# NTU-CompHydroMet-Lab/P2I-GAN-benchmark

Hardware: AMD Instinct MI355X
Metric: train frames/sec (128x128x16) (higher is better)
Workload: dtype f32

## Files before the change

### include/p2i_hip.h

```cpp
#ifndef P2I_HIP_H
#define P2I_HIP_H
#include <stdint.h>

#ifdef __cplusplus
extern "C" {
#endif

#define P2I_OK 0
#define P2I_EINVAL (-1)
#define P2I_ELDS (-2)

#define P2I_ACT_NONE 0
#define P2I_ACT_RELU 1
#define P2I_ACT_LEAKY 2
#define P2I_ACT_TANH 3

int p2i_abi_version(void);
const char* p2i_last_error(void);

typedef struct {
  int B, Cin, Cout;
  int Ti, Hi, Wi;
  int To, Ho, Wo;
  int kt, kh, kw;
// ... 4 lines not shown
int p2i_conv_fwd(const p2i_conv_desc* d, const float* x, const float* wp, const float* bias,
                 const float* residual, float* y, int act, void* stream);
int p2i_conv_dgrad(const p2i_conv_desc* d, const float* dy, const float* y_act, int act,
                   const float* wp_d, const float* dx_add, const float* mask_y, int mask_act,
                   float* dx, void* stream);
int p2i_conv_wgrad(const p2i_conv_desc* d, const float* x, const float* dy, const float* y_act,
                   int act, float* dwp, float* dbias, void* stream);
int p2i_conv_wgrad_ws(const p2i_conv_desc* d, const float* x, const float* dy, const float* y_act, int act, float* dwp,
                      float* dbias, float* ws, int64_t ws_floats, void* stream);
int p2i_conv_fwd_x6(const p2i_conv_desc* d, const float* x, const float* wp, uint16_t* wsplit, const float* bias,
                    const float* residual, float* y, int act, void* stream);
int p2i_conv_dgrad_x6(const p2i_conv_desc* d, const float* dy, const float* wp_d, uint16_t* wsplit, const float* dx_add,
                      const float* mask_y, int mask_act, float* dx, void* stream);
int p2i_x6_split(const float* wp, uint16_t* wb, int ntaps, int K, int Mpad, void* stream);
int p2i_x6_split_batched(const float* const* wp, uint16_t* const* wb, const int* ntaps, const int* K, const int* Mpad, int n,
                         void* stream);
int p2i_x6c_would_take(const p2i_conv_desc* d, int dgrad, int act);
int p2i_conv_fwd_x6s(const p2i_conv_desc* d, const float* x, const float* wp, const uint16_t* wb_layer, int ntaps_w,
                     const float* bias, const float* residual, float* y, int act, void* stream);
int p2i_conv_dgrad_x6s(const p2i_conv_desc* d, const float* dy, const float* wp_d, const uint16_t* wb_layer, int ntaps_w,
                       const float* dx_add, const float* mask_y, int mask_act, float* dx, void* stream);
int p2i_conv_last_plan(int* out6);
int p2i_fast_div_magic(int d, uint32_t* magic);
int p2i_wgrad_last_plan(int* out4);

int p2i_doconv_fold_fwd(const float* W, const float* D, const float* D_diag, int O, int I, int groups,
                        int ksz, int identity_rep, float* wp_f, float* wp_d, void* stream);
int p2i_doconv_fold_bwd(const float* dwp_f, const float* W, const float* D, const float* D_diag,
                        int O, int I, int groups, int ksz, float* dW, float* dD, void* stream);

int p2i_doconv_fold_fwd_batched(const float* const* W, const float* const* D, const float* const* D_diag, int n, int O, int I,
                                float* const* wp_f, float* const* wp_d, void* stream);
int p2i_doconv_fold_bwd_batched(const float* const* dwp_f, const float* const* W, const float* const* D,
                                const float* const* D_diag, int n, int O, int I, float* const* dW, float* const* dD,
                                void* stream);

int p2i_weight_pack(const float* w, int O, int I, int ntaps, const float* inv_div_ptr,
                    float* wp_f, float* wp_d, void* stream);
int p2i_weight_unpack_grad(const float* dwp_f, int O, int I, int ntaps, const float* w_orig,
                           const float* sigma_ptr, const float* u, const float* v, float* scratch,
                           float* dw, void* stream);

int p2i_weight_pack_batched(const float* const* w, const int* O, const int* I, const int* ntaps, const float* const* inv_div,
                            float* const* wp_f, float* const* wp_d, int n, void* stream);
int p2i_weight_unpack_grad_batched(const float* const* dwp_f, const int* O, const int* I, const int* ntaps,
                                   const float* const* w_orig, const float* const* sigma, const float* const* u,
// ... 284 lines not shown
```

### p2i-gan-benchmark_amd/csrc/conv_x6c.hip

```cpp
#include "conv_common.h"

namespace p2i {

#ifdef P2I_STAMP
extern __device__ unsigned long long* p2i_stamp_buf;
#define X6C_NOW(v) do { __builtin_amdgcn_sched_barrier(0); asm volatile("s_memtime %0\n\ts_waitcnt lgkmcnt(0)" : "=s"(v) :: "memory"); __builtin_amdgcn_sched_barrier(0); } while (0)
#define X6C_ACC(sum, t_prev) do { unsigned long long t_; X6C_NOW(t_); sum += t_ - t_prev; t_prev = t_; } while (0)
#else
#define X6C_NOW(v) do { } while (0)
#define X6C_ACC(sum, t_prev) do { } while (0)
#endif

typedef __bf16 bf16x8c __attribute__((ext_vector_type(8)));
typedef unsigned u32x4c __attribute__((ext_vector_type(4)));

__device__ __forceinline__ unsigned pack_hi16c(float lo_elem, float hi_elem) {
  return __builtin_amdgcn_perm(__float_as_uint(hi_elem), __float_as_uint(lo_elem), 0x07060302u);
}
__device__ __forceinline__ float trunc_bf16c(float v) { return __uint_as_float(__float_as_uint(v) & 0xFFFF0000u); }
__device__ __forceinline__ void split8c(const float (&v)[8], u32x4c& hi, u32x4c& mid, u32x4c& lo) {
#pragma unroll
  for (int j = 0; j < 4; ++j) {
    const float a = v[2 * j], b = v[2 * j + 1];
    hi[j] = pack_hi16c(a, b);
// ... 63 lines not shown
  const int blocks = total > 0 ? (total + 255) / 256 : 1;
  P2I_LAUNCH(wsplit_kernel, dim3(blocks > 2048 ? 2048 : blocks), dim3(256), 0, s, wp, reinterpret_cast<u32x4c*>(wb), ntaps, Ck, CmPad);
  return launch_status();
}

struct X6cGeom {
  const float* src; float* dst; const uint16_t* wb; const float* bias; const float* res; const float* mask_y;
  unsigned wb_bytes;
  int act_epi, mask_act;
  int B, Ck, Cm, CmPad;
  int sH, sW, dT, dH, dW, nH, nW;
  int ljb, ljh, ljw, eH, eW, CSl, bH, bW, nth, ntw;
  unsigned mg_ew, mg_eh;
  int ntaps_w, ksplit;
  int sT, nT, mT, oT, pT, ns, sdt0, sdt1, sdt2, swt0, swt1, swt2;
  int tap_off[9];
  int tap_w[9];
  int fused_atomic;
  int stagger;
  int vec4_epi;
  const u32x4c* splanes;
  unsigned plane_units;
  int cons_prio;
};

__device__ constexpr int X6C_CLS[9] = {3, 3, 3, 3, 2, 2, 1, 1, 0};

template <int NW> struct X6cTile {
  static constexpr int MAXCSL = NW == 8 ? 384 : 256;
  static constexpr int NI = (2 * MAXCSL + 64 * NW - 1) / (64 * NW);
};

#define X6C_WAIT1(b) asm volatile("s_waitcnt vmcnt(%0)" ::"n"(b) : "memory")
#define X6C_WAIT2(b) if (n < (b) + 1) { X6C_WAIT1(b); } else { X6C_WAIT1((b) + 1); }
#define X6C_WAIT4(b) if (n < (b) + 2) { X6C_WAIT2(b) } else { X6C_WAIT2((b) + 2) }
#define X6C_WAIT8(b) if (n < (b) + 4) { X6C_WAIT4(b) } else { X6C_WAIT4((b) + 4) }
#define X6C_WAIT16(b) if (n < (b) + 8) { X6C_WAIT8(b) } else { X6C_WAIT8((b) + 8) }
#define X6C_WAIT32(b) if (n < (b) + 16) { X6C_WAIT16(b) } else { X6C_WAIT16((b) + 16) }
__device__ __forceinline__ void x6c_wait_vm(int n) {
  if (n < 0 || n > 62) n = 0;
  if (n < 32) { X6C_WAIT32(0) } else { X6C_WAIT32(32) }
}

template <int NW, int TM, bool FUSED = false, int TPS = 3>
__global__ __launch_bounds__(64 * NW) void patch_gemm_x6c_kernel(const X6cGeom g) {
  constexpr int NCLS = FUSED ? 4 : 1;
  constexpr int NSTG = 9 / TPS;
// ... 300 lines not shown
#endif
}


template <int TM, int TPS, bool FUSED = false, bool EPI4 = false, int NPW = 4, int TN = 2, bool PRE = false>
__global__ __launch_bounds__(64 * (4 + NPW)) void patch_gemm_x6p_kernel(const X6cGeom g) {
  constexpr int NSTG = 9 / TPS;
  constexpr int NCLS = FUSED ? 4 : 1;
  static_assert(TPS == 3 || TPS == 9, "taps per stage");
  extern __shared__ __attribute__((aligned(16))) float smem[];
  constexpr int MB = 32 * TM, NCW = 4, NTHR = 64 * (NCW + NPW), NPT = 64 * NPW;
  constexpr int NI = (2 * (TN == 2 ? X6cTile<8>::MAXCSL : X6cTile<4>::MAXCSL) + NPT - 1) / NPT;
  constexpr int RING = TPS == 9 ? 3 : (TM == 2 ? 4 : 6), LEAD = RING - 1;
  constexpr int WST = 6 * TPS * MB, NWI = WST / 64;
  const int CSl = g.CSl;
  int* ptab = reinterpret_cast<int*>(smem);
  const int ptab_sz = (CSl + 3) & ~3;
  u32x4c* wbuf = reinterpret_cast<u32x4c*>(smem + ptab_sz);
  u32x4c* planes = wbuf + RING * WST;
  const int PST = 6 * CSl;

  const int tid = threadIdx.x, lane = tid & 63, wave = __builtin_amdgcn_readfirstlane(tid >> 6);
  const int l31 = lane & 31, lhi = lane >> 5;
  int tile = blockIdx.x;
  const int tw = tile % g.ntw; tile /= g.ntw;
  const int th = tile % g.nth;
  const int tb = tile / g.nth;
  const int j0b = tb << g.ljb, j0h = th << g.ljh, j0w = tw << g.ljw;
  const int o0 = blockIdx.y * MB;
  const int JWm = (1 << g.ljw) - 1, JHm = (1 << g.ljh) - 1;
  const int sHW = g.sH * g.sW;
  const int src_h0 = j0h + g.bH, src_w0 = j0w + g.bW;
  const int KCt = g.Ck >> 3;
  const int cps = g.Ck >> 4;
  const int cs = g.sT * sHW;
  const int nimg = g.B * g.nT;
  const int c0 = blockIdx.z * ((g.ns * cps) / g.ksplit);
  const int nch = (g.ns * cps) / g.ksplit;
  const int nst = NSTG * nch;

  for (int e = tid; e < CSl; e += NTHR) {
    const int row = fast_div(e, g.mg_ew);
    const int ew = e - row * g.eW;
    const int jb = fast_div(row, g.mg_eh);
    const int eh = row - jb * g.eH;
    const int n = j0b + jb, h = src_h0 + eh, w = src_w0 + ew;
    const int b = n / g.nT, lt = n - b * g.nT;
    ptab[e] = (n < nimg && (unsigned)h < (unsigned)g.sH && (unsigned)w < (unsigned)g.sW) ? ((b * (PRE ? KCt : g.Ck)) * g.sT + lt * g.mT) * sHW + h * g.sW + w : -1;
  }
  __syncthreads();

#ifdef P2I_STAMP
// ... 398 lines not shown
#ifdef P2I_STAMP
  if (p2i_stamp_buf && lane == 0) {
    asm volatile("s_waitcnt vmcnt(0)" ::: "memory");
    unsigned long long st_end; X6C_NOW(st_end);
    unsigned long long* o = p2i_stamp_buf + ((size_t)(blockIdx.x + gridDim.x * blockIdx.y) * 8 + wave) * 8;
    o[0] = st_a; o[1] = st_d; o[2] = st_b; o[3] = st_c; o[4] = st_l1 - st_l0; o[5] = st_l0 - st_entry; o[6] = st_e; o[7] = st_end - st_l1;
  }
#endif
}

static bool x6c_on() { return P2I_ENV_ONCE("P2I_CONV_X6C", 1) != 0; }
static bool x6c_fused_on() { return P2I_ENV_ONCE("P2I_CONV_X6C_FUSED", 1) != 0; }
static int x6c_min_wg() { return env_int("P2I_X6C_MIN_WG", 200); }
static int x6c_min_wg_low() { return env_int("P2I_X6C_MIN_WG", env_int("P2I_X6C_MIN_WG_LOW", 64)); }
static int x6c_fused_min_wg() { return env_int("P2I_X6C_MIN_WG", 128); }
static int x6p_tn1() { return env_int("P2I_X6P_TN1", 1); }
static int x6c_forced() { return env_int("P2I_X6C_TILE", 0); }
static int x6c_stagger() { return env_int("P2I_X6C_STAGGER", 0); }
static int x6c_fused_ksplit() { return env_int("P2I_X6C_FUSED_KSPLIT", 0); }
static int x6p_npw() { return env_int("P2I_X6P_NPW", 8) == 4 ? 4 : 8; }
static int x6c_pc() { return env_int("P2I_X6C_PC", 1); }
static int x6c_tps1() { return env_int("P2I_X6C_TPS", 9) == 3 ? 3 : 9; }
static int x6p_prio() { return env_int("P2I_X6P_PRIO", 0); }

struct X6cVariant { int NW, TM; };
static const X6cVariant kX6cVariants[] = {{8, 2}, {8, 1}, {4, 1}};

struct X6cPick { int v, jb, jh, jw, csl, ksplit; long long wgs; };
static X6cPick x6c_pick(int B, int nH, int nW, int Cm, int Ck, bool linear_epi, int Ck_slice) {
  int forced = x6c_forced();
  const int min_wg = x6c_min_wg();
  const bool tn1_ok = x6c_pc() && Ck_slice >= 32;
  if (forced == 41 && !tn1_ok) forced = 81;
  const int ksplit_on = P2I_ENV_ONCE("P2I_X6C_KSPLIT", 1);
  static const int order_a[5][2] = {{0, 0}, {1, 0}, {2, 0}, {1, 1}, {0, 1}}, order_b[5][2] = {{0, 0}, {0, 1}, {1, 0}, {2, 0}, {1, 1}};
  X6cPick low{-1, 0, 0, 0, 0, 1, 0};
  for (int cand = 0; cand < 5; ++cand) {
      const int v = (ksplit_on == 2 ? order_b : order_a)[cand][0], pass = (ksplit_on == 2 ? order_b : order_a)[cand][1];
      const X6cVariant& t = kX6cVariants[v];
      if (v == 2 && (!tn1_ok || (forced ? forced != 41 : !x6p_tn1()))) continue;
      if (forced && forced != t.NW * 10 + t.TM) continue;
      if (t.TM == 2 && Cm <= 32 && !forced) continue;
      if (pass == 1 && ((ksplit_on != 2 && t.TM != 1) || !ksplit_on || !linear_epi || ((Ck >> 4) & 1) || forced)) continue;
      int jb, jt, jh, jw;
      pick_tile_dims(32 * t.NW, B, 1, nH, nW, jb, jt, jh, jw);
      const int csl = jb * (jh + 2) * (jw + 2);
// ... 73 lines not shown
  k.wb_bytes = (2u * (unsigned)ntaps_w + (unsigned)tw_max + 1u) * (unsigned)g.Ck * (unsigned)g.CmPad * 2u;
  k.act_epi = g.act_epi; k.mask_act = g.mask_act;
  k.B = g.B; k.Ck = g.Ck; k.Cm = g.Cm; k.CmPad = g.CmPad;
  k.sH = g.sH; k.sW = g.sW; k.dT = g.dT; k.dH = g.dH; k.dW = g.dW; k.nH = c0.nH; k.nW = c0.nW;
  k.ljb = ilog2(pk.jb); k.ljh = ilog2(pk.jh); k.ljw = ilog2(pk.jw);
  k.eH = pk.jh + halo; k.eW = pk.jw + halo; k.CSl = pk.csl;
  k.nth = ceil_div(c0.nH, pk.jh); k.ntw = ceil_div(c0.nW, pk.jw);
  k.mg_ew = magic_u16(k.eW); k.mg_eh = magic_u16(k.eH);
  k.ntaps_w = ntaps_w; k.ksplit = pk.ksplit;
  k.sT = g.sT; k.nT = c0.nT; k.mT = c0.mT; k.oT = c0.oT; k.pT = c0.pT; k.ns = ns;
  k.stagger = x6c_stagger(); k.cons_prio = x6p_prio();
  return k;
}

template <void (*KERN)(const X6cGeom), int NTHR>
static void x6c_launch(const X6cGeom& k, dim3 grid, size_t lds, hipStream_t s) {
  static bool attr_set = false;
  if (!attr_set) {
    (void)hipFuncSetAttribute((const void*)KERN, hipFuncAttributeMaxDynamicSharedMemorySize, 160 * 1024);
    attr_set = true;
  }
  P2I_LAUNCH(KERN, grid, dim3(NTHR), lds, s, k);
}
static void x6c_dispatch(const X6cGeom& k, const X6cVariant& tv, int tps, bool fused, int* plan6, hipStream_t s) {
  const size_t lds = x6c_lds_bytes(k.CSl, tv.TM, tps);
  const dim3 grid((unsigned)(ceil_div(k.B * k.nT, 1 << k.ljb) * k.nth * k.ntw), (unsigned)ceil_div(k.Cm, 32 * tv.TM), (unsigned)k.ksplit);
  const bool pc = x6c_pc() && k.Ck >= 32 && (!fused || tps == 9);
  if (plan6) { plan6[0] = 32 * tv.TM; plan6[1] = 32 * tv.NW; plan6[2] = k.ksplit; plan6[3] = pc ? 4 : 8; plan6[4] = tps; plan6[5] = fused ? 8 : 7; }
  const bool pre = k.splanes != nullptr;
  if (!fused && pc) {
    if (tv.TM == 2) {
      if (k.vec4_epi) x6c_launch<patch_gemm_x6p_kernel<2, 3, false, true>, 512>(k, grid, lds, s);
      else x6c_launch<patch_gemm_x6p_kernel<2, 3>, 512>(k, grid, lds, s);
    } else if (tv.NW == 4) {
      if (pre) x6c_launch<patch_gemm_x6p_kernel<1, 9, false, false, 8, 1, true>, 768>(k, grid, lds, s);
      else x6c_launch<patch_gemm_x6p_kernel<1, 9, false, false, 8, 1>, 768>(k, grid, lds, s);
    } else if (tps == 9) {
      if (pre && x6p_npw() == 8) x6c_launch<patch_gemm_x6p_kernel<1, 9, false, false, 8, 2, true>, 768>(k, grid, lds, s);
      else if (x6p_npw() == 8) x6c_launch<patch_gemm_x6p_kernel<1, 9, false, false, 8>, 768>(k, grid, lds, s);
      else x6c_launch<patch_gemm_x6p_kernel<1, 9>, 512>(k, grid, lds, s);
    } else x6c_launch<patch_gemm_x6p_kernel<1, 3>, 512>(k, grid, lds, s);
  } else if (!fused) {
    if (tv.TM == 2) x6c_launch<patch_gemm_x6c_kernel<8, 2>, 512>(k, grid, lds, s);
    else if (tps == 9) x6c_launch<patch_gemm_x6c_kernel<8, 1, false, 9>, 512>(k, grid, lds, s);
    else x6c_launch<patch_gemm_x6c_kernel<8, 1>, 512>(k, grid, lds, s);
  } else if (pc) x6c_launch<patch_gemm_x6p_kernel<1, 9, true>, 512>(k, grid, lds, s);
  else if (tps == 9) x6c_launch<patch_gemm_x6c_kernel<8, 1, true, 9>, 512>(k, grid, lds, s);
  else x6c_launch<patch_gemm_x6c_kernel<8, 1, true>, 512>(k, grid, lds, s);
}

// ... 123 lines not shown
  for (int i = 0; i < n; ++i) {
    P2I_REQUIRE(wp[i] && wb[i] && ntaps[i] > 0 && K[i] > 0 && (K[i] & 7) == 0 && Mpad[i] > 0 && (Mpad[i] & 31) == 0, "p2i_x6_split_batched: bad tensor %d", i);
    b.wp[i] = wp[i]; b.wb[i] = reinterpret_cast<u32x4c*>(wb[i]); b.ntaps[i] = ntaps[i]; b.Ck[i] = K[i]; b.CmPad[i] = Mpad[i];
    const int tot = ntaps[i] * (K[i] >> 3) * Mpad[i];
    if (tot > maxn) maxn = tot;
  }
  const int blocks = (maxn + 255) / 256;
  P2I_LAUNCH(wsplit_batched_kernel, dim3(blocks > 1024 ? 1024 : blocks, n), dim3(256), 0, (hipStream_t)stream, b);
  return launch_status();
}

extern "C" int p2i_x6_split_planes(const float* x, void* planes, int B, int C, int64_t P, void* stream) {
  P2I_REQUIRE(x && planes && B > 0 && C > 0 && (C & 7) == 0 && P > 0, "split planes: C % 8 == 0");
  const long long total = (long long)B * (C >> 3) * P;
  const long long blocks = (total + 255) / 256;
  P2I_LAUNCH(p2i::split_planes_kernel, dim3((unsigned)(blocks > 8192 ? 8192 : blocks)), dim3(256), 0, (hipStream_t)stream, x,
             static_cast<p2i::u32x4c*>(planes), B, C >> 3, (long long)P);
  return p2i::launch_status();
}
extern "C" int p2i_x6_next_source_planes(const void* planes) {
  p2i::g_next_splanes = planes;
  return P2I_OK;
}
```

### p2i-gan-benchmark_amd/csrc/wgrad_x6.hip

```cpp
#include "conv_common.h"

namespace p2i {

#ifdef P2I_STAMP
extern __device__ unsigned long long* p2i_stamp_buf;
#define WX_NOW(v) do { __builtin_amdgcn_sched_barrier(0); asm volatile("s_memtime %0\n\ts_waitcnt lgkmcnt(0)" : "=s"(v) :: "memory"); __builtin_amdgcn_sched_barrier(0); } while (0)
#else
#define WX_NOW(v) do { } while (0)
#endif

typedef short s16x4w __attribute__((ext_vector_type(4)));
typedef __bf16 bf16x8w __attribute__((ext_vector_type(8)));
typedef unsigned u32x4w __attribute__((ext_vector_type(4)));
typedef float f32x4w __attribute__((ext_vector_type(4)));

struct Wx6Geom {
  const float* x;
  const float* dy;
  float* dwp;
  float* partial;
  float* dbias;
  long long pstride;
  long long bias_off;
  int B, Cx, Co, CoPad, H, W;
// ... 18 lines not shown
#pragma unroll
  for (int j = 0; j < 4; ++j) {
    const float a = v[2 * j], b = v[2 * j + 1];
    hi[j] = wx_pack(a, b);
    const float ra = a - wx_trunc(a), rb = b - wx_trunc(b);
    mid[j] = wx_pack(ra, rb);
    const float sa = ra - wx_trunc(ra), sb = rb - wx_trunc(rb);
    lo[j] = wx_pack(sa, sb);
  }
}

typedef __attribute__((address_space(3))) s16x4w* lds_s16x4_ptr;
__device__ __forceinline__ bf16x8w wx_read_tr(const unsigned char* base, int byte_off) {
  const s16x4w a = __builtin_amdgcn_ds_read_tr16_b64_v4i16((lds_s16x4_ptr)(base + byte_off));
  const s16x4w b = __builtin_amdgcn_ds_read_tr16_b64_v4i16((lds_s16x4_ptr)(base + byte_off + 4 * WX_ROW));
  return __builtin_bit_cast(bf16x8w, __builtin_shufflevector(a, b, 0, 1, 2, 3, 4, 5, 6, 7));
}
__device__ __forceinline__ bf16x8w wx_read_tr_s4(const unsigned char* base, int byte_off) {
  const s16x4w a = __builtin_amdgcn_ds_read_tr16_b64_v4i16((lds_s16x4_ptr)(base + byte_off));
  const s16x4w b = __builtin_amdgcn_ds_read_tr16_b64_v4i16((lds_s16x4_ptr)(base + byte_off + WX_ROW));
  return __builtin_bit_cast(bf16x8w, __builtin_shufflevector(a, b, 0, 1, 2, 3, 4, 5, 6, 7));
}

template <bool S4, int DIAG = 0>
__global__ __launch_bounds__(512) void wgrad_x6_kernel(const Wx6Geom g) {
  extern __shared__ __attribute__((aligned(16))) unsigned char wsm[];
#ifdef P2I_STAMP
  unsigned long long st_entry, st_loop0 = 0, st_loop1 = 0, st_bar = 0, st_t;
  WX_NOW(st_entry);
#endif
  const int tid = threadIdx.x, lane = tid & 63, wave = __builtin_amdgcn_readfirstlane(tid >> 6);
  const int tg = wave >> 2, kh = (wave >> 1) & 1, mh = wave & 1;
  const int i16 = lane & 15, g16 = (lane >> 4) & 1, lhi = lane >> 5, l31 = lane & 31;
  const int HW = g.H * g.W;
  const int cb = blockIdx.y, ob = blockIdx.z % g.nco, ta = blockIdx.z / g.nco;
  const int dta = ta == 2 ? g.dt[2] : (ta == 1 ? g.dt[1] : g.dt[0]);
  const int xcs = g.sT * HW, ycs = g.nT * HW;

  int x_rel[WX_NXI], x_dst[WX_NXI], x_qr[WX_NXI], x_qc[WX_NXI];
#pragma unroll
  for (int it = 0; it < WX_NXI; ++it) {
    const int e = tid + 512 * it;
    const bool in = e < 8 * WX_XPX;
    const int chunk = in ? e / WX_XPX : 0, q = in ? e - chunk * WX_XPX : 0;
    const int qr = q / WX_EW, qc = q - qr * WX_EW;
    x_qr[it] = in ? qr - 1 : -(1 << 20);
    x_qc[it] = qc - 1;
    x_rel[it] = (cb * 64 + chunk * 8) * xcs + (qr - 1) * g.W + (qc - 1);
// ... 3 lines not shown
  const int y_rel = (ob * 64 + y_chunk * 8) * ycs + (y_q >> 4) * g.W + (y_q & 15);
  const int y_dst = WX_YOFF + y_q * WX_ROW + y_chunk * 16;

  float sv[3][8];
  const __amdgpu_buffer_rsrc_t rs_x = __builtin_amdgcn_make_buffer_rsrc(const_cast<float*>(g.x), 0, (int)g.x_bytes, 0x00020000);
  const __amdgpu_buffer_rsrc_t rs_y = __builtin_amdgcn_make_buffer_rsrc(const_cast<float*>(g.dy), 0, (int)g.dy_bytes, 0x00020000);
  unsigned so[3];
  const bool x1_in = tid + 512 < 8 * WX_XPX;
  const int dummy_dst = 2 * WX_BUF + lane * 16;
  auto tile_ptrs = [&](int t) {
    const int tw = t % g.ntw, r0 = t / g.ntw;
    const int th = r0 % g.nth, img = r0 / g.nth;
    const int b = img / g.nT, to = img - b * g.nT;
    const int ti = to * g.mT + dta;
    const bool tok = (unsigned)ti < (unsigned)g.sT;
    const int h0 = th * WX_TH, w0 = tw * WX_TW;
    const int xorg = (b * g.Cx * g.sT + ti) * HW + h0 * g.W + w0, yorg = (b * g.Co * g.nT + to) * HW + h0 * g.W + w0;
#pragma unroll
    for (int it = 0; it < WX_NXI; ++it) {
      const int h = h0 + x_qr[it], w = w0 + x_qc[it];
      const bool ok = tok && (unsigned)h < (unsigned)g.H && (unsigned)w < (unsigned)g.W;
      so[it] = ok ? 4u * (unsigned)(xorg + x_rel[it]) : 0xFFFFFF00u;
    }
    so[2] = 4u * (unsigned)(yorg + y_rel);
  };
  const int xchan_bytes = 4 * xcs, ychan_bytes = 4 * ycs;
  auto load_chunk = [&](int c) {
#pragma unroll
    for (int f = 3 * c; f < 3 * c + 3; ++f)
      sv[f >> 3][f & 7] = __builtin_bit_cast(float, __builtin_amdgcn_raw_buffer_load_b32((f >> 3) == 2 ? rs_y : rs_x, so[f >> 3],
                                                                                      (f & 7) * ((f >> 3) == 2 ? ychan_bytes : xchan_bytes), 0));
  };
  const bool do_bias = g.dbias != nullptr && cb == 0 && ta == 0;
  float bsum[8] = {0.f, 0.f, 0.f, 0.f, 0.f, 0.f, 0.f, 0.f};
  float bias_w = 1.f;
  auto split_chunk = [&](int c, unsigned char* buf) {
    const int it = c / 3, pl = c % 3;
    float (&v)[8] = sv[it];
    if (c == 6 && do_bias) {
#pragma unroll
      for (int j = 0; j < 8; ++j) bsum[j] += bias_w * v[j];
    }
    u32x4w w;
#pragma unroll
    for (int j = 0; j < 4; ++j) w[j] = wx_pack(v[2 * j], v[2 * j + 1]);
    const int dst = it == 2 ? y_dst + pl * WX_YPLANE : (it == 1 && !x1_in ? -1 : x_dst[it] + pl * WX_XPLANE);
    *reinterpret_cast<u32x4w*>(dst < 0 ? wsm + dummy_dst : buf + dst) = w;
    if (pl < 2) {
#pragma unroll
      for (int j = 0; j < 8; ++j) v[j] = v[j] - wx_trunc(v[j]);
    }
  };

  f32x16 acc[5];
#pragma unroll
  for (int t = 0; t < 5; ++t)
#pragma unroll
    for (int r = 0; r < 16; ++r) acc[t][r] = 0.f;

  const int lrow = S4 ? 2 * lhi + 4 * (i16 >> 2) : 8 * lhi + (i16 >> 2);
  const int a_lane = lrow * WX_ROW + (32 * kh + 16 * g16 + 4 * (i16 & 3)) * 2;
  const int b_lane = WX_YOFF + lrow * WX_ROW + (32 * mh + 16 * g16 + 4 * (i16 & 3)) * 2;
  int a_tap[5];
#pragma unroll
  for (int k = 0; k < 4; ++k) {
    const int tap = 5 * tg + k;
    a_tap[k] = a_lane + ((tap / 3) * WX_EW + tap % 3) * WX_ROW;
  }
  a_tap[4] = a_lane + (WX_EW + 1) * WX_ROW;
  int rowx[WX_TH], rowy[WX_TH];
#pragma unroll
  for (int ks = 0; ks < WX_TH; ++ks) {
    const int row = (ks + 2 * tg) & 3;
    rowx[ks] = row * WX_EW * WX_ROW;
    rowy[ks] = row * WX_TW * WX_ROW;
  }
  constexpr int NSTEP = 18;
  constexpr int ST_KS[NSTEP] = {0, 0, 0, 0, 0, 1, 1, 1, 1, 1, 2, 2, 2, 2, 3, 3, 3, 3};
  constexpr int ST_K[NSTEP] = {0, 1, 2, 3, 4, 0, 1, 2, 3, 4, 0, 1, 2, 3, 0, 1, 2, 3};

  constexpr int PA[6] = {2, 0, 1, 1, 0, 0};
  constexpr int PB[6] = {0, 2, 1, 0, 1, 0};

  int t = blockIdx.x;
  if (t < g.ntiles) {
    tile_ptrs(t);
#pragma unroll
    for (int c = 0; c < 8; ++c) load_chunk(c);
#pragma unroll
    for (int c = 0; c < 9; ++c) split_chunk(c, wsm);
  }
  __syncthreads();
  int cur = 0;
  WX_NOW(st_loop0);
  for (; t < g.ntiles; t += gridDim.x) {
    const int tn = t + gridDim.x;
    const bool more = tn < g.ntiles;
    tile_ptrs(more ? tn : t);
    bias_w = more ? 1.f : 0.f;
    const unsigned char* buf = wsm + cur * WX_BUF;
    unsigned char* nbuf = wsm + (cur ^ 1) * WX_BUF;
    bf16x8w Av[3][3], Bv[2][3];
    auto load_a = [&](int set, int step) {
      const unsigned char* p = buf + a_tap[ST_K[step]] + rowx[ST_KS[step]];
#pragma unroll
      for (int pl = 0; pl < 3; ++pl) Av[set][pl] = S4 ? wx_read_tr_s4(p, pl * WX_XPLANE) : wx_read_tr(p, pl * WX_XPLANE);
    };
    auto load_b = [&](int set, int ks) {
      const unsigned char* p = buf + b_lane + rowy[ks];
#pragma unroll
      for (int pl = 0; pl < 3; ++pl) Bv[set][pl] = S4 ? wx_read_tr_s4(p, pl * WX_YPLANE) : wx_read_tr(p, pl * WX_YPLANE);
    };
    load_b(0, 0);
    load_a(0, 0);
    load_a(1, 1);
    __builtin_amdgcn_sched_barrier(0);
#pragma unroll
    for (int i = 0; i < NSTEP; ++i) {
      const int ks = ST_KS[i], k = ST_K[i];
      const bool pre_a = i + 2 < NSTEP;
      const bool pre_b = ks + 1 < WX_TH && (i == 0 || ST_KS[i - 1] != ks);
      if (i < 8 && !(DIAG & 1)) load_chunk(i);
      if (i >= 9 && !(DIAG & 2)) split_chunk(i - 9, nbuf);
      if (pre_a && !(DIAG & 8)) load_a((i + 2) % 3, i + 2);
      if (pre_b && !(DIAG & 8)) load_b((ks + 1) & 1, ks + 1);
      if (!(DIAG & 4)) {
#pragma unroll
        for (int q = 0; q < 6; ++q)
          acc[k] = __builtin_amdgcn_mfma_f32_32x32x16_bf16(Av[i % 3][PA[q]], Bv[ks & 1][PB[q]], acc[k], 0, 0, 0);
      } else {
#pragma unroll
        for (int pl = 0; pl < 3; ++pl) asm volatile("" :: "v"(Av[i % 3][pl]), "v"(Bv[ks & 1][pl]));
      }
#pragma unroll
      for (int q = 0; q < 6; ++q) {
        __builtin_amdgcn_sched_group_barrier(0x008, 1, 0);
        if (pre_a && pre_b) __builtin_amdgcn_sched_group_barrier(0x100, 2, 0);
        else if (pre_a || pre_b) __builtin_amdgcn_sched_group_barrier(0x100, 1, 0);
        if (i < 8 && q < 3) { __builtin_amdgcn_sched_group_barrier(0x002, 2, 0); __builtin_amdgcn_sched_group_barrier(0x020, 1, 0); }
        if (i >= 9) __builtin_amdgcn_sched_group_barrier(0x002, 4, 0);
        if (i >= 9 && q == 5) __builtin_amdgcn_sched_group_barrier(0x200, 1, 0);
      }
      __builtin_amdgcn_sched_barrier(0);
    }
#ifdef P2I_STAMP
    WX_NOW(st_t);
#endif
    __syncthreads();
#ifdef P2I_STAMP
    { unsigned long long t2; WX_NOW(t2); st_bar += t2 - st_t; }
#endif
    cur ^= 1;
  }
  WX_NOW(st_loop1);

  f32x4w* red = reinterpret_cast<f32x4w*>(wsm);
  const int quad = kh * 2 + mh;
  if (tg == 1) {
#pragma unroll
    for (int j4 = 0; j4 < 4; ++j4) {
      f32x4w v;
#pragma unroll
      for (int e = 0; e < 4; ++e) v[e] = acc[4][4 * j4 + e];
      red[(quad * 4 + j4) * 64 + lane] = v;
    }
  }
  __syncthreads();
  if (tg == 0) {
#pragma unroll
    for (int j4 = 0; j4 < 4; ++j4) {
      const f32x4w v = red[(quad * 4 + j4) * 64 + lane];
#pragma unroll
      for (int e = 0; e < 4; ++e) acc[4][4 * j4 + e] += v[e];
    }
  }
  const size_t tap_stride = (size_t)g.Cx * g.CoPad;
  float* dst = (g.partial ? g.partial + (size_t)blockIdx.x * g.pstride : g.dwp) + (size_t)ta * 9 * tap_stride +
               ((size_t)cb * 64 + 32 * kh + 4 * lhi) * g.CoPad + ob * 64 + 32 * mh + l31;
  if (do_bias) {
#pragma unroll
    for (int j = 0; j < 8; ++j) {
      const float sj = wave_sum(bsum[j]);
      if (lane == 0) {
        if (g.partial) g.partial[(size_t)blockIdx.x * g.pstride + g.bias_off + ob * 64 + y_chunk * 8 + j] = sj;
        else atomicAdd(g.dbias + ob * 64 + y_chunk * 8 + j, sj);
      }
    }
  }
  auto emit = [&](auto&& put) {
#pragma unroll
    for (int k = 0; k < 5; ++k) {
      if (k == 4 && tg == 1) break;
      float* dt = dst + (k == 4 ? 4 : 5 * tg + k) * tap_stride;
#pragma unroll
      for (int j = 0; j < 16; ++j) put(dt + ((j & 3) + 8 * (j >> 2)) * g.CoPad, acc[k][j]);
    }
  };
  if (g.partial) emit([](float* o, float v) { *o = v; });
  else emit([](float* o, float v) { atomicAdd(o, v); });
#ifdef P2I_STAMP
  if (p2i_stamp_buf && lane == 0) {
    asm volatile("s_waitcnt vmcnt(0)" ::: "memory");
    unsigned long long st_end; WX_NOW(st_end);
    unsigned long long* o = p2i_stamp_buf + ((size_t)(blockIdx.x + gridDim.x * (blockIdx.y + gridDim.y * blockIdx.z)) * 8 + wave) * 8;
    o[0] = st_loop0 - st_entry; o[1] = st_loop1 - st_loop0; o[2] = st_end - st_loop1; o[3] = st_bar; o[4] = st_entry; o[5] = st_end;
  }
#endif
}


__global__ __launch_bounds__(512) void wgrad_x6p_kernel(const Wx6Geom g) {
  extern __shared__ __attribute__((aligned(16))) unsigned char wsm[];
  const int tid = threadIdx.x, lane = tid & 63, wave = __builtin_amdgcn_readfirstlane(tid >> 6);
  const int HW = g.H * g.W;
  const int cb = blockIdx.y, ob = blockIdx.z % g.nco, ta = blockIdx.z / g.nco;
  const int dta = ta == 2 ? g.dt[2] : (ta == 1 ? g.dt[1] : g.dt[0]);
  const int xcs = g.sT * HW, ycs = g.nT * HW;
  const int nmine = blockIdx.x < g.ntiles ? (g.ntiles - 1 - (int)blockIdx.x) / (int)gridDim.x + 1 : 0;
// ... 159 lines not shown
  }
  const size_t tap_stride = (size_t)g.Cx * g.CoPad;
  float* dst = (g.partial ? g.partial + (size_t)blockIdx.x * g.pstride : g.dwp) + (size_t)ta * 9 * tap_stride +
               ((size_t)cb * 64 + 32 * kh + 4 * lhi) * g.CoPad + ob * 64 + 32 * mh + l31;
#pragma unroll
  for (int tp = 0; tp < 9; ++tp) {
    float* dt = dst + tp * tap_stride;
#pragma unroll
    for (int j = 0; j < 16; ++j) {
      float* o = dt + ((j & 3) + 8 * (j >> 2)) * g.CoPad;
      if (g.partial) *o = acc[tp][j];
      else atomicAdd(o, acc[tp][j]);
    }
  }
}

int run_wgrad_x6(const p2i_conv_desc* d, const float* x, const float* dy, float* dwp, float* dbias, float* ws, long long ws_floats,
                 int* ns_out, long long* slice_out, hipStream_t s) {
  if (env_int("P2I_WGRAD_X6", 1) == 0) return 1;
  if (d->kh != 3 || d->kw != 3 || d->sh != 1 || d->sw != 1 || d->ph != 1 || d->pw != 1) return 1;
  const bool flat = d->kt == 1 && d->st == 1 && d->pt == 0;
  const bool vol = d->kt == 3 && d->pt == 1 && d->st <= 2;
  if (!flat && !vol) return 1;
  if ((d->Cin & 63) || (d->Cout & 63) || (d->Wo % WX_TW) || (d->Ho % WX_TH)) return 1;
  const long long nx = (long long)d->B * d->Cin * d->Ti * d->Hi * d->Wi, ny = (long long)d->B * d->Cout * d->To * d->Ho * d->Wo;
  if (nx >= (1ll << 30) - 64 || ny >= (1ll << 30) - 64) return 1;
  Wx6Geom g{};
  g.x = x; g.dy = dy; g.dwp = dwp; g.dbias = dbias;
  g.B = d->B; g.Cx = d->Cin; g.Co = d->Cout; g.CoPad = (d->Cout + 31) / 32 * 32; g.H = d->Ho; g.W = d->Wo;
  g.x_bytes = (unsigned)(4 * nx); g.dy_bytes = (unsigned)(4 * ny);
  g.sT = d->Ti; g.nT = d->To; g.mT = d->st;
  for (int a = 0; a < d->kt; ++a) g.dt[a] = a - d->pt;
  g.nth = d->Ho / WX_TH; g.ntw = d->Wo / WX_TW; g.ntiles = d->B * d->To * g.nth * g.ntw;
  const int ncb = d->Cin / 64, nco = d->Cout / 64;
  g.nco = nco;
  int ns = 256 / (ncb * nco * d->kt);
  if (ns < 1) ns = 1;
  if (ns > g.ntiles) ns = g.ntiles;
  const long long slice = 9ll * d->kt * d->Cin * g.CoPad;
  const long long pstr = slice + (dbias ? g.CoPad : 0);
  const bool sliced = ns >= 2 && ws != nullptr && pstr * ns <= ws_floats && slice < (1ll << 31);
  if (ns >= 2 && !sliced) return 1;
  g.partial = sliced ? ws : nullptr;
  g.pstride = pstr;
  g.bias_off = slice;
  static bool attr_set = false;
  if (!attr_set) {
    (void)hipFuncSetAttribute((const void*)wgrad_x6_kernel<false>, hipFuncAttributeMaxDynamicSharedMemorySize, 160 * 1024);
    (void)hipFuncSetAttribute((const void*)wgrad_x6_kernel<true>, hipFuncAttributeMaxDynamicSharedMemorySize, 160 * 1024);
    (void)hipFuncSetAttribute((const void*)wgrad_x6p_kernel, hipFuncAttributeMaxDynamicSharedMemorySize, 160 * 1024);
    attr_set = true;
  }
  if (env_int("P2I_WGRAD_X6_PC", 0) != 0) P2I_LAUNCH(wgrad_x6p_kernel, dim3(ns, ncb, nco * d->kt), dim3(512), 2 * WX_BUF + 1024, s, g);
#ifdef P2I_STAMP
  else if (const int dg = env_int("P2I_WGRAD_DIAG", 0)) {
    const dim3 gr(ns, ncb, nco * d->kt);
#define WX_DIAG_CASE(n) case n: { static bool a_ = false; if (!a_) { (void)hipFuncSetAttribute((const void*)wgrad_x6_kernel<true, n>, hipFuncAttributeMaxDynamicSharedMemorySize, 160 * 1024); a_ = true; } \
      P2I_LAUNCH((wgrad_x6_kernel<true, n>), gr, dim3(512), 2 * WX_BUF + 1024, s, g); break; }
    switch (dg) { WX_DIAG_CASE(1) WX_DIAG_CASE(2) WX_DIAG_CASE(3) WX_DIAG_CASE(4) WX_DIAG_CASE(8) WX_DIAG_CASE(12) WX_DIAG_CASE(11) WX_DIAG_CASE(7)
      default: P2I_LAUNCH(wgrad_x6_kernel<true>, gr, dim3(512), 2 * WX_BUF + 1024, s, g); }
#undef WX_DIAG_CASE
  }
#endif
  else if (env_int("P2I_WGRAD_X6_S4", 1) != 0)
    P2I_LAUNCH(wgrad_x6_kernel<true>, dim3(ns, ncb, nco * d->kt), dim3(512), 2 * WX_BUF + 1024, s, g);
  else P2I_LAUNCH(wgrad_x6_kernel<false>, dim3(ns, ncb, nco * d->kt), dim3(512), 2 * WX_BUF + 1024, s, g);
  *ns_out = sliced ? ns : 0;
  *slice_out = slice;
  return launch_status();
}

}
```

### p2i-gan-benchmark_amd/p2igan_bench/_hip.py

```python
from __future__ import annotations

import ctypes as C
import os

_LIB_PATH = os.path.join(os.path.dirname(os.path.abspath(__file__)), "_lib", "libp2i_hip.so")
_lib = None

ACT_NONE, ACT_RELU, ACT_LEAKY, ACT_TANH = 0, 1, 2, 3


class ConvDesc(C.Structure):
    _fields_ = [(n, C.c_int) for n in
                ("B", "Cin", "Cout", "Ti", "Hi", "Wi", "To", "Ho", "Wo", "kt", "kh", "kw",
                 "st", "sh", "sw", "pt", "ph", "pw")]


_P = C.c_void_p
_I = C.c_int
_F = C.c_float
_L = C.c_int64
_F64 = C.c_double
_D = C.POINTER(ConvDesc)

SIGNATURES = {
    "p2i_conv_fwd": [_D, _P, _P, _P, _P, _P, _I, _P],
    "p2i_conv_dgrad": [_D, _P, _P, _I, _P, _P, _P, _I, _P, _P],
    "p2i_conv_wgrad": [_D, _P, _P, _P, _I, _P, _P, _P],
    "p2i_conv_wgrad_ws": [_D, _P, _P, _P, _I, _P, _P, _P, _L, _P],
    "p2i_conv_fwd_x6": [_D, _P, _P, _P, _P, _P, _P, _I, _P],
    "p2i_conv_dgrad_x6": [_D, _P, _P, _P, _P, _P, _I, _P, _P],
    "p2i_x6_split": [_P, _P, _I, _I, _I, _P],
    "p2i_x6_split_batched": [_P, _P, _P, _P, _P, _I, _P],
    "p2i_x6c_would_take": [_D, _I, _I],
    "p2i_conv_fwd_x6s": [_D, _P, _P, _P, _I, _P, _P, _P, _I, _P],
    "p2i_conv_dgrad_x6s": [_D, _P, _P, _P, _I, _P, _P, _I, _P, _P],
    "p2i_conv_last_plan": [C.POINTER(C.c_int)],
    "p2i_wgrad_last_plan": [C.POINTER(C.c_int)],
    "p2i_fast_div_magic": [_I, C.POINTER(C.c_uint32)],
    "p2i_doconv_fold_fwd": [_P, _P, _P, _I, _I, _I, _I, _I, _P, _P, _P],
    "p2i_doconv_fold_bwd": [_P, _P, _P, _P, _I, _I, _I, _I, _P, _P, _P],
    "p2i_doconv_fold_fwd_batched": [_P, _P, _P, _I, _I, _I, _P, _P, _P],
    "p2i_doconv_fold_bwd_batched": [_P, _P, _P, _P, _I, _I, _I, _P, _P, _P],
    "p2i_weight_pack": [_P, _I, _I, _I, _P, _P, _P, _P],
    "p2i_weight_pack_batched": [_P, _P, _P, _P, _P, _P, _P, _I, _P],
    "p2i_weight_unpack_grad_batched": [_P, _P, _P, _P, _P, _P, _P, _P, _P, _P, _I, _P],
    "p2i_weight_unpack_grad_batched_acc": [_P, _P, _P, _P, _P, _P, _P, _P, _P, _P, _I, _I, _P],
    "p2i_weight_unpack_grad": [_P, _I, _I, _I, _P, _P, _P, _P, _P, _P, _P],
    "p2i_spectral_norm": [_P, _I, _I, _P, _P, _I, _P, _P, _P],
    "p2i_spectral_norm_batched": [_P, _P, _P, _P, _P, _I, _P, _P, _P, _P, _I, _P],
    "p2i_attn_fwd": [_P, _P, _P, _P, _P, _P, _I, _I, _I, _P],
    "p2i_attn_bwd": [_P, _P, _P, _P, _P, _P, _P, _P, _P, _P, _I, _I, _I, _P],
    "p2i_idw_fwd": [_P, _P, _P, _P, _P, _P, _P, _P, _P, _P, _P, _P, _P, _I, _I, _I, _I, _F, _P],
    "p2i_idw_fwd_ws": [_P, _P, _P, _P, _P, _P, _P, _P, _P, _P, _P, _P, _P, _P, _I, _I, _I, _I, _F, _P],
    "p2i_idw_bwd": [_P, _P, _P, _P, _P, _P, _I, _I, _I, _I, _P],
    "p2i_pooldup_fwd": [_P, _P, _I, _I, _I, _I, _P],
    "p2i_pooldup_bwd": [_P, _P, _P, _I, _I, _I, _I, _P],
    "p2i_upmod_fwd": [_P, _P, _P, _I, _I, _I, _I, _P],
    "p2i_window_gather": [_P, _P, _P, _P, _I, _L, _I, _I, _I, _I, _P],
    "p2i_window_mean": [_P, _P, _I, _L, _I, _I, _I, _F, _P],
    "p2i_upmod_fwd_ba": [_P, _P, _P, _I, _P, _I, _I, _I, _I, _P],
    "p2i_upmod_bwd": [_P, _P, _P, _P, _P, _I, _I, _I, _I, _P],
# ... 146 lines not shown
```

Before: 12060.

## Use 16x16x32 MFMA in wgrad, allow ragged tiles, add XCD-aware tile ordering

The weight-gradient kernel gains a 16x16x32 bf16 MFMA variant with its own LDS lane mapping, accumulator layout and instruction schedule, and it becomes the default. Wgrad is also extended to output shapes that are not multiples of the tile size, using bounds-masked dy offsets, so more layers can take this path. Separately, an opt-in XCD-aware block remapping for the patch-GEMM forward is added, off by default, to improve L2 reuse of weights and source data across chiplets. The new MFMA shape changes register pressure and the issue pattern, and the ragged-tile path adds masking work.

```diff
diff --git a/include/p2i_hip.h b/include/p2i_hip.h
--- a/include/p2i_hip.h
+++ b/include/p2i_hip.h
@@ -50,6 +50,8 @@
                        const float* dx_add, const float* mask_y, int mask_act, float* dx, void* stream);
 int p2i_conv_last_plan(int* out6);
 int p2i_fast_div_magic(int d, uint32_t* magic);
+int p2i_x6p_tile_order(int ntiles, int ncm, int64_t w_bytes, int64_t s_bytes, int force, int* a_out);
+int p2i_x6p_tile_decode(int ntiles, int ncm, int a, int* tile_out, int* cm_out);
 int p2i_wgrad_last_plan(int* out4);
 
 int p2i_doconv_fold_fwd(const float* W, const float* D, const float* D_diag, int O, int I, int groups,
diff --git a/p2i-gan-benchmark_amd/csrc/conv_x6c.hip b/p2i-gan-benchmark_amd/csrc/conv_x6c.hip
--- a/p2i-gan-benchmark_amd/csrc/conv_x6c.hip
+++ b/p2i-gan-benchmark_amd/csrc/conv_x6c.hip
@@ -109,7 +109,22 @@
   const u32x4c* splanes;
   unsigned plane_units;
   int cons_prio;
+  int ord_nt, ord_a;
 };
+
+__host__ __device__ __forceinline__ void x6p_tile_decode(int id, int nt, int ncm, int a, int& tile, int& cm) {
+  if (a <= 0) {
+    cm = id / nt;
+    tile = id - cm * nt;
+    return;
+  }
+  const int nwg = nt * ncm, q = nwg >> 3, r = nwg & 7, c = id & 7;
+  const int L = (c < r ? c * (q + 1) : r * (q + 1) + (c - r) * q) + (id >> 3);
+  const int p = L / (a * nt), rem = L - p * a * nt;
+  const int wa = ncm - p * a < a ? ncm - p * a : a;
+  tile = rem / wa;
+  cm = p * a + rem - tile * wa;
+}
 
 __device__ constexpr int X6C_CLS[9] = {3, 3, 3, 3, 2, 2, 1, 1, 0};
 
@@ -456,12 +471,13 @@
 
   const int tid = threadIdx.x, lane = tid & 63, wave = __builtin_amdgcn_readfirstlane(tid >> 6);
   const int l31 = lane & 31, lhi = lane >> 5;
-  int tile = blockIdx.x;
+  int tile = blockIdx.x, cmt = blockIdx.y;
+  if (!FUSED && g.ord_nt) x6p_tile_decode((int)blockIdx.x, g.ord_nt, (g.Cm + MB - 1) / MB, g.ord_a, tile, cmt);
   const int tw = tile % g.ntw; tile /= g.ntw;
   const int th = tile % g.nth;
   const int tb = tile / g.nth;
   const int j0b = tb << g.ljb, j0h = th << g.ljh, j0w = tw << g.ljw;
-  const int o0 = blockIdx.y * MB;
+  const int o0 = cmt * MB;
   const int JWm = (1 << g.ljw) - 1, JHm = (1 << g.ljh) - 1;
   const int sHW = g.sH * g.sW;
   const int src_h0 = j0h + g.bH, src_w0 = j0w + g.bW;
@@ -906,6 +922,21 @@
 static int x6c_pc() { return env_int("P2I_X6C_PC", 1); }
 static int x6c_tps1() { return env_int("P2I_X6C_TPS", 9) == 3 ? 3 : 9; }
 static int x6p_prio() { return env_int("P2I_X6P_PRIO", 0); }
+static int x6p_xcd() { return env_int("P2I_X6P_XCD", 0); }
+
+static int x6p_tile_order(int nt, int ncm, long long w_bytes, long long s_bytes, bool force) {
+  int g8 = 8;
+  while (nt % g8) g8 >>= 1;
+  auto lim = [](int v, int hi) { return v < hi ? v : hi; };
+  const long long ident = w_bytes * lim(8, nt) + s_bytes * lim(8 / g8, ncm);
+  long long best = -1;
+  int best_a = 0;
+  for (int gc = 8; gc >= 1; gc >>= 1) {
+    const long long cost = w_bytes * lim(8 / gc, nt) + s_bytes * lim(gc, ncm);
+    if (best < 0 || cost < best) { best = cost; best_a = ceil_div(ncm, lim(gc, ncm)); }
+  }
+  return (force || 4 * best <= 3 * ident) ? best_a : 0;
+}
 
 struct X6cVariant { int NW, TM; };
 static const X6cVariant kX6cVariants[] = {{8, 2}, {8, 1}, {4, 1}};
@@ -1025,10 +1056,20 @@
   }
   P2I_LAUNCH(KERN, grid, dim3(NTHR), lds, s, k);
 }
-static void x6c_dispatch(const X6cGeom& k, const X6cVariant& tv, int tps, bool fused, int* plan6, hipStream_t s) {
+static void x6c_dispatch(const X6cGeom& k_in, const X6cVariant& tv, int tps, bool fused, int* plan6, hipStream_t s) {
+  X6cGeom k = k_in;
   const size_t lds = x6c_lds_bytes(k.CSl, tv.TM, tps);
-  const dim3 grid((unsigned)(ceil_div(k.B * k.nT, 1 << k.ljb) * k.nth * k.ntw), (unsigned)ceil_div(k.Cm, 32 * tv.TM), (unsigned)k.ksplit);
+  dim3 grid((unsigned)(ceil_div(k.B * k.nT, 1 << k.ljb) * k.nth * k.ntw), (unsigned)ceil_div(k.Cm, 32 * tv.TM), (unsigned)k.ksplit);
   const bool pc = x6c_pc() && k.Ck >= 32 && (!fused || tps == 9);
+  const int xcd = x6p_xcd();
+  if (xcd != 0 && !fused && pc && k.ksplit == 1 && (long long)grid.x * grid.y < (1ll << 30)) {
+    const int a = x6p_tile_order((int)grid.x, (int)grid.y, 6ll * 9 * k.ns * k.Ck * k.CmPad, 4ll * k.B * k.Ck * k.sT * k.sH * k.sW, xcd == 2);
+    if (a > 0) {
+      k.ord_nt = (int)grid.x;
+      k.ord_a = a;
+      grid = dim3(grid.x * grid.y, 1, 1);
+    }
+  }
   if (plan6) { plan6[0] = 32 * tv.TM; plan6[1] = 32 * tv.NW; plan6[2] = k.ksplit; plan6[3] = pc ? 4 : 8; plan6[4] = tps; plan6[5] = fused ? 8 : 7; }
   const bool pre = k.splanes != nullptr;
   if (!fused && pc) {
@@ -1198,3 +1239,15 @@
   p2i::g_next_splanes = planes;
   return P2I_OK;
 }
+
+extern "C" int p2i_x6p_tile_order(int ntiles, int ncm, int64_t w_bytes, int64_t s_bytes, int force, int* a_out) {
+  P2I_REQUIRE(a_out != nullptr && ntiles >= 1 && ncm >= 1 && w_bytes >= 0 && s_bytes >= 0, "p2i_x6p_tile_order: bad arguments");
+  *a_out = p2i::x6p_tile_order(ntiles, ncm, w_bytes, s_bytes, force != 0);
+  return P2I_OK;
+}
+extern "C" int p2i_x6p_tile_decode(int ntiles, int ncm, int a, int* tile_out, int* cm_out) {
+  P2I_REQUIRE(tile_out && cm_out && ntiles >= 1 && ncm >= 1 && a >= 0 && a <= ncm && (long long)ntiles * ncm < (1ll << 30),
+              "p2i_x6p_tile_decode: bad arguments");
+  for (int id = 0; id < ntiles * ncm; ++id) p2i::x6p_tile_decode(id, ntiles, ncm, a, tile_out[id], cm_out[id]);
+  return P2I_OK;
+}
diff --git a/p2i-gan-benchmark_amd/csrc/wgrad_x6.hip b/p2i-gan-benchmark_amd/csrc/wgrad_x6.hip
--- a/p2i-gan-benchmark_amd/csrc/wgrad_x6.hip
+++ b/p2i-gan-benchmark_amd/csrc/wgrad_x6.hip
@@ -64,8 +64,9 @@
   return __builtin_bit_cast(bf16x8w, __builtin_shufflevector(a, b, 0, 1, 2, 3, 4, 5, 6, 7));
 }
 
-template <bool S4, int DIAG = 0>
+template <bool S4, int DIAG = 0, int MSHAPE = 32>
 __global__ __launch_bounds__(512) void wgrad_x6_kernel(const Wx6Geom g) {
+  static_assert(MSHAPE == 32 || (MSHAPE == 16 && S4), "MFMA shape: 32x32x16, or 16x16x32 with the conflict-free rows");
   extern __shared__ __attribute__((aligned(16))) unsigned char wsm[];
 #ifdef P2I_STAMP
   unsigned long long st_entry, st_loop0 = 0, st_loop1 = 0, st_bar = 0, st_t;
@@ -115,7 +116,7 @@
       const bool ok = tok && (unsigned)h < (unsigned)g.H && (unsigned)w < (unsigned)g.W;
       so[it] = ok ? 4u * (unsigned)(xorg + x_rel[it]) : 0xFFFFFF00u;
     }
-    so[2] = 4u * (unsigned)(yorg + y_rel);
+    so[2] = (h0 + (y_q >> 4) < g.H && w0 + (y_q & 15) < g.W) ? 4u * (unsigned)(yorg + y_rel) : 0xFFFFFF00u;
   };
   const int xchan_bytes = 4 * xcs, ychan_bytes = 4 * ycs;
   auto load_chunk = [&](int c) {
@@ -145,15 +146,26 @@
     }
   };
 
-  f32x16 acc[5];
-#pragma unroll
-  for (int t = 0; t < 5; ++t)
-#pragma unroll
-    for (int r = 0; r < 16; ++r) acc[t][r] = 0.f;
+  f32x16 acc[MSHAPE == 32 ? 5 : 1];
+  f32x4w acc4[MSHAPE == 16 ? 20 : 1];
+  if constexpr (MSHAPE == 32) {
+#pragma unroll
+    for (int t = 0; t < 5; ++t)
+#pragma unroll
+      for (int r = 0; r < 16; ++r) acc[t][r] = 0.f;
+  } else {
+#pragma unroll
+    for (int t = 0; t < 20; ++t)
+#pragma unroll
+      for (int r = 0; r < 4; ++r) acc4[t][r] = 0.f;
+  }
 
   const int lrow = S4 ? 2 * lhi + 4 * (i16 >> 2) : 8 * lhi + (i16 >> 2);
-  const int a_lane = lrow * WX_ROW + (32 * kh + 16 * g16 + 4 * (i16 & 3)) * 2;
-  const int b_lane = WX_YOFF + lrow * WX_ROW + (32 * mh + 16 * g16 + 4 * (i16 & 3)) * 2;
+  const int lcol16 = 8 * g16 + 2 * (i16 >> 2);
+  const int a_lane = MSHAPE == 16 ? (lhi * WX_EW + lcol16) * WX_ROW + (32 * kh + 4 * (i16 & 3)) * 2
+                                  : lrow * WX_ROW + (32 * kh + 16 * g16 + 4 * (i16 & 3)) * 2;
+  const int b_lane = MSHAPE == 16 ? WX_YOFF + (lhi * WX_TW + lcol16) * WX_ROW + (32 * mh + 4 * (i16 & 3)) * 2
+                                  : WX_YOFF + lrow * WX_ROW + (32 * mh + 16 * g16 + 4 * (i16 & 3)) * 2;
   int a_tap[5];
 #pragma unroll
   for (int k = 0; k < 4; ++k) {
@@ -161,16 +173,19 @@
     a_tap[k] = a_lane + ((tap / 3) * WX_EW + tap % 3) * WX_ROW;
   }
   a_tap[4] = a_lane + (WX_EW + 1) * WX_ROW;
-  int rowx[WX_TH], rowy[WX_TH];
-#pragma unroll
-  for (int ks = 0; ks < WX_TH; ++ks) {
-    const int row = (ks + 2 * tg) & 3;
+  constexpr int NKS = MSHAPE == 16 ? 2 : WX_TH;
+  int rowx[NKS], rowy[NKS];
+#pragma unroll
+  for (int ks = 0; ks < NKS; ++ks) {
+    const int row = MSHAPE == 16 ? 2 * ((ks + tg) & 1) : (ks + 2 * tg) & 3;
     rowx[ks] = row * WX_EW * WX_ROW;
     rowy[ks] = row * WX_TW * WX_ROW;
   }
   constexpr int NSTEP = 18;
   constexpr int ST_KS[NSTEP] = {0, 0, 0, 0, 0, 1, 1, 1, 1, 1, 2, 2, 2, 2, 3, 3, 3, 3};
   constexpr int ST_K[NSTEP] = {0, 1, 2, 3, 4, 0, 1, 2, 3, 4, 0, 1, 2, 3, 0, 1, 2, 3};
+  constexpr int SS_KS[NSTEP] = {0, 0, 0, 0, 0, 0, 0, 0, 0, 0, 1, 1, 1, 1, 1, 1, 1, 1};
+  constexpr int SS_K[NSTEP] = {0, 0, 1, 1, 2, 2, 3, 3, 4, 4, 0, 0, 1, 1, 2, 2, 3, 3};
 
   constexpr int PA[6] = {2, 0, 1, 1, 0, 0};
   constexpr int PB[6] = {0, 2, 1, 0, 1, 0};
@@ -193,6 +208,7 @@
     bias_w = more ? 1.f : 0.f;
     const unsigned char* buf = wsm + cur * WX_BUF;
     unsigned char* nbuf = wsm + (cur ^ 1) * WX_BUF;
+    if constexpr (MSHAPE == 32) {
     bf16x8w Av[3][3], Bv[2][3];
     auto load_a = [&](int set, int step) {
       const unsigned char* p = buf + a_tap[ST_K[step]] + rowx[ST_KS[step]];
@@ -236,6 +252,56 @@
       }
       __builtin_amdgcn_sched_barrier(0);
     }
+    } else {
+    bf16x8w Av[3][3], Bv[2][2][3];
+    auto load_a = [&](int set, int step) {
+      const unsigned char* p = buf + a_tap[SS_K[step]] + rowx[SS_KS[step]] + 32 * (step & 1);
+#pragma unroll
+      for (int pl = 0; pl < 3; ++pl) Av[set][pl] = wx_read_tr_s4(p, pl * WX_XPLANE);
+    };
+    auto load_b = [&](int set, int ks) {
+#pragma unroll
+      for (int mm = 0; mm < 2; ++mm) {
+        const unsigned char* p = buf + b_lane + rowy[ks] + 32 * mm;
+#pragma unroll
+        for (int pl = 0; pl < 3; ++pl) Bv[set][mm][pl] = wx_read_tr_s4(p, pl * WX_YPLANE);
+      }
+    };
+    load_b(0, 0);
+    load_a(0, 0);
+    load_a(1, 1);
+    __builtin_amdgcn_sched_barrier(0);
+#pragma unroll
+    for (int i = 0; i < NSTEP; ++i) {
+      const int ks = SS_KS[i], k = SS_K[i], kk = i & 1;
+      const bool pre_a = i + 2 < NSTEP;
+      const bool pre_b = i == 0;
+      if (i < 8 && !(DIAG & 1)) load_chunk(i);
+      if (i >= 9 && !(DIAG & 2)) split_chunk(i - 9, nbuf);
+      if (pre_a && !(DIAG & 8)) load_a((i + 2) % 3, i + 2);
+      if (pre_b && !(DIAG & 8)) load_b(1, 1);
+      if (!(DIAG & 4)) {
+#pragma unroll
+        for (int q = 0; q < 6; ++q)
+#pragma unroll
+          for (int mm = 0; mm < 2; ++mm)
+            acc4[(k * 2 + kk) * 2 + mm] = __builtin_amdgcn_mfma_f32_16x16x32_bf16(Av[i % 3][PA[q]], Bv[ks][mm][PB[q]], acc4[(k * 2 + kk) * 2 + mm], 0, 0, 0);
+      } else {
+#pragma unroll
+        for (int pl = 0; pl < 3; ++pl) asm volatile("" :: "v"(Av[i % 3][pl]), "v"(Bv[ks][0][pl]), "v"(Bv[ks][1][pl]));
+      }
+#pragma unroll
+      for (int q = 0; q < 12; ++q) {
+        __builtin_amdgcn_sched_group_barrier(0x008, 1, 0);
+        if (pre_a && !(q & 1)) __builtin_amdgcn_sched_group_barrier(0x100, 1, 0);
+        if (pre_b) __builtin_amdgcn_sched_group_barrier(0x100, 1, 0);
+        if (i < 8 && q < 3) { __builtin_amdgcn_sched_group_barrier(0x002, 2, 0); __builtin_amdgcn_sched_group_barrier(0x020, 1, 0); }
+        if (i >= 9) __builtin_amdgcn_sched_group_barrier(0x002, 2, 0);
+        if (i >= 9 && q == 11) __builtin_amdgcn_sched_group_barrier(0x200, 1, 0);
+      }
+      __builtin_amdgcn_sched_barrier(0);
+    }
+    }
 #ifdef P2I_STAMP
     WX_NOW(st_t);
 #endif
@@ -253,8 +319,11 @@
 #pragma unroll
     for (int j4 = 0; j4 < 4; ++j4) {
       f32x4w v;
-#pragma unroll
-      for (int e = 0; e < 4; ++e) v[e] = acc[4][4 * j4 + e];
+      if constexpr (MSHAPE == 16) v = acc4[16 + j4];
+      else {
+#pragma unroll
+        for (int e = 0; e < 4; ++e) v[e] = acc[4][4 * j4 + e];
+      }
       red[(quad * 4 + j4) * 64 + lane] = v;
     }
   }
@@ -264,12 +333,15 @@
     for (int j4 = 0; j4 < 4; ++j4) {
       const f32x4w v = red[(quad * 4 + j4) * 64 + lane];
 #pragma unroll
-      for (int e = 0; e < 4; ++e) acc[4][4 * j4 + e] += v[e];
+      for (int e = 0; e < 4; ++e) {
+        if constexpr (MSHAPE == 16) acc4[16 + j4][e] += v[e];
+        else acc[4][4 * j4 + e] += v[e];
+      }
     }
   }
   const size_t tap_stride = (size_t)g.Cx * g.CoPad;
   float* dst = (g.partial ? g.partial + (size_t)blockIdx.x * g.pstride : g.dwp) + (size_t)ta * 9 * tap_stride +
-               ((size_t)cb * 64 + 32 * kh + 4 * lhi) * g.CoPad + ob * 64 + 32 * mh + l31;
+               ((size_t)cb * 64 + 32 * kh + 4 * (MSHAPE == 16 ? lane >> 4 : lhi)) * g.CoPad + ob * 64 + 32 * mh + (MSHAPE == 16 ? i16 : l31);
   if (do_bias) {
 #pragma unroll
     for (int j = 0; j < 8; ++j) {
@@ -285,8 +357,14 @@
     for (int k = 0; k < 5; ++k) {
       if (k == 4 && tg == 1) break;
       float* dt = dst + (k == 4 ? 4 : 5 * tg + k) * tap_stride;
-#pragma unroll
-      for (int j = 0; j < 16; ++j) put(dt + ((j & 3) + 8 * (j >> 2)) * g.CoPad, acc[k][j]);
+      if constexpr (MSHAPE == 16) {
+#pragma unroll
+        for (int j = 0; j < 16; ++j)
+          put(dt + (16 * (j >> 3) + (j & 3)) * g.CoPad + 16 * ((j >> 2) & 1), acc4[(k * 2 + (j >> 3)) * 2 + ((j >> 2) & 1)][j & 3]);
+      } else {
+#pragma unroll
+        for (int j = 0; j < 16; ++j) put(dt + ((j & 3) + 8 * (j >> 2)) * g.CoPad, acc[k][j]);
+      }
     }
   };
   if (g.partial) emit([](float* o, float v) { *o = v; });
@@ -492,7 +570,9 @@
   const bool flat = d->kt == 1 && d->st == 1 && d->pt == 0;
   const bool vol = d->kt == 3 && d->pt == 1 && d->st <= 2;
   if (!flat && !vol) return 1;
-  if ((d->Cin & 63) || (d->Cout & 63) || (d->Wo % WX_TW) || (d->Ho % WX_TH)) return 1;
+  if ((d->Cin & 63) || (d->Cout & 63)) return 1;
+  const int pc_on = env_int("P2I_WGRAD_X6_PC", 0);
+  if (pc_on && ((d->Wo % WX_TW) || (d->Ho % WX_TH))) return 1;
   const long long nx = (long long)d->B * d->Cin * d->Ti * d->Hi * d->Wi, ny = (long long)d->B * d->Cout * d->To * d->Ho * d->Wo;
   if (nx >= (1ll << 30) - 64 || ny >= (1ll << 30) - 64) return 1;
   Wx6Geom g{};
@@ -501,7 +581,7 @@
   g.x_bytes = (unsigned)(4 * nx); g.dy_bytes = (unsigned)(4 * ny);
   g.sT = d->Ti; g.nT = d->To; g.mT = d->st;
   for (int a = 0; a < d->kt; ++a) g.dt[a] = a - d->pt;
-  g.nth = d->Ho / WX_TH; g.ntw = d->Wo / WX_TW; g.ntiles = d->B * d->To * g.nth * g.ntw;
+  g.nth = ceil_div(d->Ho, WX_TH); g.ntw = ceil_div(d->Wo, WX_TW); g.ntiles = d->B * d->To * g.nth * g.ntw;
   const int ncb = d->Cin / 64, nco = d->Cout / 64;
   g.nco = nco;
   int ns = 256 / (ncb * nco * d->kt);
@@ -518,10 +598,11 @@
   if (!attr_set) {
     (void)hipFuncSetAttribute((const void*)wgrad_x6_kernel<false>, hipFuncAttributeMaxDynamicSharedMemorySize, 160 * 1024);
     (void)hipFuncSetAttribute((const void*)wgrad_x6_kernel<true>, hipFuncAttributeMaxDynamicSharedMemorySize, 160 * 1024);
+    (void)hipFuncSetAttribute((const void*)wgrad_x6_kernel<true, 0, 16>, hipFuncAttributeMaxDynamicSharedMemorySize, 160 * 1024);
     (void)hipFuncSetAttribute((const void*)wgrad_x6p_kernel, hipFuncAttributeMaxDynamicSharedMemorySize, 160 * 1024);
     attr_set = true;
   }
-  if (env_int("P2I_WGRAD_X6_PC", 0) != 0) P2I_LAUNCH(wgrad_x6p_kernel, dim3(ns, ncb, nco * d->kt), dim3(512), 2 * WX_BUF + 1024, s, g);
+  if (pc_on != 0) P2I_LAUNCH(wgrad_x6p_kernel, dim3(ns, ncb, nco * d->kt), dim3(512), 2 * WX_BUF + 1024, s, g);
 #ifdef P2I_STAMP
   else if (const int dg = env_int("P2I_WGRAD_DIAG", 0)) {
     const dim3 gr(ns, ncb, nco * d->kt);
@@ -532,9 +613,11 @@
 #undef WX_DIAG_CASE
   }
 #endif
-  else if (env_int("P2I_WGRAD_X6_S4", 1) != 0)
-    P2I_LAUNCH(wgrad_x6_kernel<true>, dim3(ns, ncb, nco * d->kt), dim3(512), 2 * WX_BUF + 1024, s, g);
-  else P2I_LAUNCH(wgrad_x6_kernel<false>, dim3(ns, ncb, nco * d->kt), dim3(512), 2 * WX_BUF + 1024, s, g);
+  else if (env_int("P2I_WGRAD_X6_S4", 1) != 0) {
+    if (env_int("P2I_WGRAD_X6_MFMA", 16) != 32)
+      P2I_LAUNCH((wgrad_x6_kernel<true, 0, 16>), dim3(ns, ncb, nco * d->kt), dim3(512), 2 * WX_BUF + 1024, s, g);
+    else P2I_LAUNCH(wgrad_x6_kernel<true>, dim3(ns, ncb, nco * d->kt), dim3(512), 2 * WX_BUF + 1024, s, g);
+  } else P2I_LAUNCH(wgrad_x6_kernel<false>, dim3(ns, ncb, nco * d->kt), dim3(512), 2 * WX_BUF + 1024, s, g);
   *ns_out = sliced ? ns : 0;
   *slice_out = slice;
   return launch_status();
diff --git a/p2i-gan-benchmark_amd/p2igan_bench/_hip.py b/p2i-gan-benchmark_amd/p2igan_bench/_hip.py
--- a/p2i-gan-benchmark_amd/p2igan_bench/_hip.py
+++ b/p2i-gan-benchmark_amd/p2igan_bench/_hip.py
@@ -37,6 +37,8 @@
     "p2i_conv_last_plan": [C.POINTER(C.c_int)],
     "p2i_wgrad_last_plan": [C.POINTER(C.c_int)],
     "p2i_fast_div_magic": [_I, C.POINTER(C.c_uint32)],
+    "p2i_x6p_tile_order": [_I, _I, _L, _L, _I, C.POINTER(C.c_int)],
+    "p2i_x6p_tile_decode": [_I, _I, _I, C.POINTER(C.c_int), C.POINTER(C.c_int)],
     "p2i_doconv_fold_fwd": [_P, _P, _P, _I, _I, _I, _I, _I, _P, _P, _P],
     "p2i_doconv_fold_bwd": [_P, _P, _P, _P, _I, _I, _I, _I, _P, _P, _P],
     "p2i_doconv_fold_fwd_batched": [_P, _P, _P, _I, _I, _I, _P, _P, _P],
```

Measured after the change: 11940. 0.99x the previous value.
